# IXarea/LittleGAN

Measured on AMD Instinct MI355X. Metric: 128x128 CelebA-shaped images/sec (G+D+Adj step), higher is better.
Workload: dtype bf16; 1 GPU; C3: 128x128x3 synthetic CelebA, batch 256/GPU, bf16 MFMA conv/transposed-conv + Adjuster branch; global_batch=256, per_gpu_batch=256, image=128, cond_dim=40, parallelism=dp1, launch=eager launches

## Files before the change

### littlegan_amd/csrc/conv_up4.hip

```cpp
#include <type_traits>
#include "lg_internal.h"

namespace {

constexpr int TH = 8, TW = 16, HHT = TH + 2, HWT = TW + 2, NPX = HHT * HWT;
constexpr int KC = 64, KS = KC / 16;
constexpr int PITCH = KC * 2 + 16;
constexpr int HB = 32768;
constexpr int PHW = 10, PNPX = 100, PS1 = 104;
template <bool PAIR> struct U4L {
  static constexpr int HWP = PAIR ? PHW : HWT;
  static constexpr int NPIECE = (PAIR ? 2 * PNPX : NPX) * (KC / 8);
  static constexpr int PPT = (NPIECE + 255) / 256;
};
static_assert((PS1 + PNPX) * PITCH <= HB, "pair halo fits the buffer");
constexpr int SRED_OFF = 2 * HB, SBIAS_OFF = 2 * HB + 256, LDS_BYTES = 2 * HB + 256 + 512;

struct U4Params {
  const __bf16* src;
  const char* wp;
  const float* bias;
  __bf16* out;
  double* spart;
  int B, Hs, Ws, Cs, N, N32, KB;
  int tpi_x, tpi, ntn, nper, nparts;
  int ga, gb;
  LgNormFuse nf;
};

__device__ __forceinline__ int pix32(int r) {
  const int q = r >> 2, lo = r & 3;
  const int odd = (q ^ (q >> 1) ^ (q >> 2)) & 1;
  const int rank = odd ? ((q == 1) ? 0 : (q == 2) ? 1 : (q == 4) ? 2 : 3) : ((q == 0) ? 0 : (q == 3) ? 1 : (q == 5) ? 2 : 3);
  return odd * 16 + rank * 4 + lo;
}

constexpr int nk(int p) { return p ? 3 : 2; }
constexpr int ntaps_of(int cls) { return nk(cls >> 1) * nk(cls & 1); }
constexpr int tap_k(int p, int a) { return p ? 2 * a : 2 * a + 1; }
constexpr int tap_d(int p, int a) { return (p + 1 - tap_k(p, a)) / 2; }
constexpr int tap_widx(int cls, int t) { return tap_k(cls >> 1, t / nk(cls & 1)) * 5 + tap_k(cls & 1, t % nk(cls & 1)); }
constexpr int tap_aoff(int cls, int t, int hwp) {
  return ((tap_d(cls >> 1, t / nk(cls & 1)) + 1) * hwp + tap_d(cls & 1, t % nk(cls & 1)) + 1) * PITCH;
}
template <int CLS, bool STATS, bool FUSE, bool PAIR>
__device__ __forceinline__ void up4_run(const U4Params& p, char* smem, int lb, int G) {
  constexpr int HWP = U4L<PAIR>::HWP, NPIECE = U4L<PAIR>::NPIECE, PPT = U4L<PAIR>::PPT;
  constexpr int F = ntaps_of(CLS) * KS;
  constexpr int RING = F % 8 == 0 ? 8 : 12;
  double* sred = reinterpret_cast<double*>(smem + SRED_OFF);
  float* sbias = reinterpret_cast<float*>(smem + SBIAS_OFF);
  const int tid = threadIdx.x, lane = tid & 63, r = lane & 31, h = lane >> 5;
  const int wid = __builtin_amdgcn_readfirstlane(tid >> 6);
  const int nmine = (p.nper - lb + G - 1) / G;
  const int nchunk = p.Cs / KC;
  const int total = nmine * nchunk;

  int pl[PPT], pyx[PPT];
#pragma unroll
  for (int u = 0; u < PPT; ++u) {
    const int q = tid + u * 256;
    pl[u] = -1; pyx[u] = 0;
    if (q < NPIECE) {
      const int px = q >> 3, pc = q & 7;
      if constexpr (PAIR) {
        const int sl = px >= PNPX, pp = px - PNPX * sl, hy = pp / PHW, hx = pp - hy * PHW;
        pl[u] = (pp + PS1 * sl) * PITCH + pc * 16;
        pyx[u] = (pc << 16) | (hy << 8) | (sl << 7) | hx;
      } else {
        const int hy = px / HWT, hx = px - hy * HWT;
        pl[u] = px * PITCH + pc * 16;
        pyx[u] = (pc << 16) | (hy << 8) | hx;
      }
    }
  }
  int abase[4];
#pragma unroll
  for (int i = 0; i < 4; ++i) {
    const int m = i * 32 + pix32(r);
    const int col = m & 15;
    abase[i] = ((m >> 4) * HWP + (PAIR ? (col & 7) + PS1 * (col >> 3) : col)) * PITCH + h * 16;
  }

  unsigned long long wzero = 0;
  struct Item { int n, y0, x0, tn; };
  auto decode = [&](int k) {
    const int rest = lb + k * G;
    Item it;
    it.tn = rest % p.ntn;
    const int tm = rest / p.ntn;
    if constexpr (PAIR) { it.n = 2 * tm; it.y0 = 0; it.x0 = 0; return it; }
    it.n = tm / p.tpi;
    const int tt = tm - it.n * p.tpi;
    it.y0 = (tt / p.tpi_x) * TH; it.x0 = (tt % p.tpi_x) * TW;
    return it;
  };
  constexpr unsigned OOB = 0x80000000u;
  const int sample_elems = p.Hs * p.Ws * p.Cs;
  auto issue = [&](const Item& it, int c0, u32x4 (&v)[PPT]) {
    const __amdgpu_buffer_rsrc_t rs = __builtin_amdgcn_make_buffer_rsrc(const_cast<__bf16*>(p.src + (long long)it.n * sample_elems), 0,
                                                                        (PAIR ? 2 : 1) * sample_elems * 2, 0x00027000);
#pragma unroll
    for (int u = 0; u < PPT; ++u) {
      const int pq = pyx[u] + (int)wzero;
      const int sy = it.y0 - 1 + ((pq >> 8) & 255), sx = it.x0 - 1 + (pq & (PAIR ? 127 : 255));
      const int sl = PAIR ? (pq >> 7) & 1 : 0;
      const bool in = pl[u] >= 0 && (unsigned)sy < (unsigned)p.Hs && (unsigned)sx < (unsigned)p.Ws;
      const unsigned off = in ? (unsigned)((((sl * p.Hs + sy) * p.Ws + sx) * p.Cs + c0 + (pq >> 16) * 8) * 2) : OOB;
      v[u] = __builtin_bit_cast(u32x4, __builtin_amdgcn_raw_buffer_load_b128(rs, off, 0, 0));
    }
  };
  auto commit = [&](char* buf, const u32x4 (&v)[PPT]) {
#pragma unroll
    for (int u = 0; u < PPT; ++u)
      if (pl[u] >= 0) *reinterpret_cast<u32x4*>(buf + pl[u]) = v[u];
  };
  const unsigned lane16 = lane * 16;
  const unsigned long long wstride = (unsigned long long)p.N32 * p.KB * 1024ull;
  auto wbase = [&](int tn, int kb) { return p.wp + ((long long)(tn * 4 + wid) * p.KB + kb) * 1024; };
  auto wfrag = [&](const char* base, int widx, int ks) {
    return *reinterpret_cast<const u32x4*>((base + ((wzero + (unsigned long long)widx) * wstride + ks * 1024)) + lane16);
  };

  f32x16 acc[4];
#pragma unroll
  for (int i = 0; i < 4; ++i)
#pragma unroll
    for (int e = 0; e < 16; ++e) acc[i][e] = 0.f;
  u32x4 bf[RING];
  u32x4 hv[PPT];

  Item cur = decode(0);
  issue(cur, 0, hv);
  {
    const char* w0 = wbase(cur.tn, 0);
#pragma unroll
    for (int f = 0; f < RING; ++f) bf[f] = wfrag(w0, tap_widx(CLS, f / KS), f % KS);
  }
  commit(smem, hv);
  auto load_bias = [&](int tn) {
    if (tid < 128) sbias[tid] = p.bias ? p.bias[tn * 128 + tid] : 0.f;
  };
  load_bias(cur.tn);
  __syncthreads();

  int k = 0, c = 0;
  Item nxt = cur;
  int c2 = 0;
  auto slice = [&](int s) {
    constexpr int OFF = 0;
    const char* hbuf = smem + (s & 1) * HB;
    const char* wcur = wbase(cur.tn, c * KS);
    const char* wnxt = wbase(nxt.tn, c2 * KS);
    bf16x8 a[2][4];
#pragma unroll
    for (int i = 0; i < 4; ++i) a[0][i] = *reinterpret_cast<const bf16x8*>(hbuf + abase[i] + tap_aoff(CLS, 0, HWP));
    __builtin_amdgcn_sched_barrier(0);
#pragma unroll
    for (int f = 0; f < F; ++f) {
      if (f + 1 < F) {
#pragma unroll
        for (int i = 0; i < 4; ++i)
          a[(f + 1) & 1][i] = *reinterpret_cast<const bf16x8*>(hbuf + abase[i] + tap_aoff(CLS, (f + 1 < F ? f + 1 : 0) / KS, HWP) + ((f + 1) % KS) * 32);
      }
      const int slot = (f + OFF) % RING;
#pragma unroll
      for (int i = 0; i < 4; ++i)
        acc[i] = __builtin_amdgcn_mfma_f32_32x32x16_bf16(__builtin_bit_cast(bf16x8, bf[slot]), a[f & 1][i], acc[i], 0, 0, 0);
      if (f + RING < F) bf[slot] = wfrag(wcur, tap_widx(CLS, (f + RING < F ? f + RING : 0) / KS), (f + RING) % KS);
      else bf[slot] = wfrag(wnxt, tap_widx(CLS, (f + RING >= F ? f + RING - F : 0) / KS), (f + RING - F) % KS);
#pragma unroll
      for (int i = 0; i < 4; ++i) {
        __builtin_amdgcn_sched_group_barrier(0x008, 1, 0);
        __builtin_amdgcn_sched_group_barrier(0x100, 1, 0);
      }
      __builtin_amdgcn_sched_group_barrier(0x020, 1, 0);
    }
    commit(smem + ((s + 1) & 1) * HB, hv);
    __syncthreads();
  };
  auto epilogue = [&](int s, bool more) {
      char* C = smem + (s & 1) * HB;
      const float shift = STATS ? sbias[0] : 0.f;
      const f32x2 shift2 = {shift, shift};
      f32x2 s1v = {0.f, 0.f}, s2v = {0.f, 0.f};
      f32x4 bq[4];
#pragma unroll
      for (int g = 0; g < 4; ++g) bq[g] = *reinterpret_cast<const f32x4*>(sbias + wid * 32 + 8 * g + 4 * h);
#pragma unroll
      for (int i = 0; i < 4; ++i) {
        const int row = i * 32 + pix32(r);
#pragma unroll
        for (int g = 0; g < 4; ++g) {
          bf16x4 w;
#pragma unroll
          for (int jj = 0; jj < 2; ++jj) {
            const f32x2 v = f32x2{acc[i][4 * g + 2 * jj], acc[i][4 * g + 2 * jj + 1]} + f32x2{bq[g][2 * jj], bq[g][2 * jj + 1]};
            if constexpr (STATS) {
              const f32x2 d = v - shift2;
              s1v += d;
              s2v = __builtin_elementwise_fma(d, d, s2v);
            }
            w[2 * jj] = (__bf16)v[0]; w[2 * jj + 1] = (__bf16)v[1];
          }
          *reinterpret_cast<bf16x4*>(C + row * 256 + (((wid * 4 + g) ^ (row & 15)) << 4) + 8 * h) = w;
        }
      }
      if constexpr (STATS) {
        const double l1 = (double)s1v[0] + (double)s1v[1], l2 = (double)s2v[0] + (double)s2v[1];
        if constexpr (PAIR) {
          const bool sb = (pix32(r) & 8) != 0;
          const double a1 = lg_wave_sum_d(sb ? 0.0 : l1), a2 = lg_wave_sum_d(sb ? 0.0 : l2);
          const double b1 = lg_wave_sum_d(sb ? l1 : 0.0), b2 = lg_wave_sum_d(sb ? l2 : 0.0);
          if (lane == 0) {
            double* q = sred + (k & 1) * 16;
            q[wid] = a1; q[4 + wid] = a2; q[8 + wid] = b1; q[12 + wid] = b2;
          }
        } else {
          const double w1 = lg_wave_sum_d(l1), w2 = lg_wave_sum_d(l2);
          if (lane == 0) { sred[(k & 1) * 16 + wid] = w1; sred[(k & 1) * 16 + 4 + wid] = w2; }
        }
      }
      constexpr int py = CLS >> 1, pxc = CLS & 1;
      const long long obase = ((long long)(cur.n * 2 * p.Hs + 2 * cur.y0 + py) * (2 * p.Ws) + 2 * cur.x0 + pxc) * p.N + cur.tn * 128;
      const long long sample_out = (long long)4 * p.Hs * p.Ws * p.N;
      auto pix_off = [&](int row) -> long long {
        if constexpr (PAIR) return obase + ((row >> 3) & 1) * sample_out + ((long long)(2 * (row >> 4)) * (2 * p.Ws) + 2 * (row & 7)) * p.N;
        else return obase + ((long long)(2 * (row >> 4)) * (2 * p.Ws) + 2 * (row & 15)) * p.N;
      };
      u32x4 zq[FUSE ? 8 : 1];
      (void)zq;
      if constexpr (FUSE) {
#pragma unroll
        for (int q8 = 0; q8 < 8; ++q8) {
          const int piece = tid + q8 * 256 + (int)wzero, row = piece >> 4, j = piece & 15;
          zq[q8] = *reinterpret_cast<const u32x4*>(p.nf.z + pix_off(row) + j * 8);
        }
      }
      __syncthreads();
      float nf1 = 0.f, nf2 = 0.f;
      (void)nf1; (void)nf2;
#pragma unroll
      for (int q8 = 0; q8 < 8; ++q8) {
        const int piece = tid + q8 * 256 + (int)wzero, row = piece >> 4, j = piece & 15;
        const u32x4 v = *reinterpret_cast<const u32x4*>(C + row * 256 + ((j ^ (row & 15)) << 4));
        *reinterpret_cast<u32x4*>(p.out + pix_off(row) + j * 8) = v;
        if constexpr (FUSE) {
          const lg_const_f32p sp = lg_as_const(p.nf.stats + (long long)(cur.n + (PAIR ? wid >> 1 : 0)) * 8);
          lg_nf_accum(v, zq[q8], lg_uniform(sp[0]), lg_uniform(sp[4]), lg_uniform(sp[2]), lg_uniform(sp[3]), p.nf.alpha, nf1, nf2);
        }
      }
      if constexpr (FUSE) {
        const double w1 = lg_wave_sum_d((double)nf1), w2 = lg_wave_sum_d((double)nf2);
        if (lane == 0) { sred[(k & 1) * 16 + wid] = w1; sred[(k & 1) * 16 + 4 + wid] = w2; }
      }
      const int tin = PAIR ? 0 : (cur.y0 / TH) * p.tpi_x + cur.x0 / TW;
      const long long prec = (long long)cur.n * p.nparts + (tin * 4 + CLS) * p.ntn + cur.tn;
      if constexpr (STATS) {
        if (tid == 0) {
          const double* q = sred + (k & 1) * 16;
          if constexpr (PAIR) {
            constexpr double cnt = 64.0 * 128.0;
#pragma unroll
            for (int sm = 0; sm < 2; ++sm) {
              const double S1 = (q[8 * sm] + q[8 * sm + 1]) + (q[8 * sm + 2] + q[8 * sm + 3]);
              const double S2 = (q[8 * sm + 4] + q[8 * sm + 5]) + (q[8 * sm + 6] + q[8 * sm + 7]);
              const double md = S1 / cnt;
              double* o = p.spart + (prec + (long long)sm * p.nparts) * 3;
              o[0] = cnt; o[1] = (double)shift + md; o[2] = S2 - cnt * md * md;
            }
          } else {
            constexpr double cnt = 128.0 * 128.0;
            const double S1 = (q[0] + q[1]) + (q[2] + q[3]), S2 = (q[4] + q[5]) + (q[6] + q[7]);
            const double md = S1 / cnt;
            double* o = p.spart + prec * 3;
            o[0] = cnt; o[1] = (double)shift + md; o[2] = S2 - cnt * md * md;
          }
        }
      }
      __syncthreads();
      if constexpr (FUSE) {
        if (tid == 0) {
          const double* q = sred + (k & 1) * 16;
          if constexpr (PAIR) {
#pragma unroll
            for (int sm = 0; sm < 2; ++sm) {
              double* o = p.nf.part + (prec + (long long)sm * p.nparts) * 2;
              o[0] = q[2 * sm] + q[2 * sm + 1]; o[1] = q[4 + 2 * sm] + q[4 + 2 * sm + 1];
            }
          } else {
            double* o = p.nf.part + prec * 2;
            o[0] = (q[0] + q[1]) + (q[2] + q[3]); o[1] = (q[4] + q[5]) + (q[6] + q[7]);
          }
        }
      }
#pragma unroll
      for (int i = 0; i < 4; ++i)
#pragma unroll
        for (int e = 0; e < 16; ++e) acc[i][e] = 0.f;
      if (more && nxt.tn != cur.tn) load_bias(nxt.tn);
      ++k;
  };
  for (int s = 0; s < total; ++s) {
    const bool more = s + 1 < total;
    const bool last_c = c + 1 == nchunk;
    nxt = cur;
    c2 = c + 1;
    if (last_c) { c2 = 0; if (more) nxt = decode(k + 1); }
    if (!more) c2 = c;
    wzero = 0;
    asm volatile("" : "+s"(wzero));
    issue(nxt, c2 * KC, hv);
    slice(s);
    if (last_c) epilogue(s, more);
    cur = nxt;
    c = c2;
  }
}

template <bool STATS, bool FUSE, bool PAIR = false>
__global__ __launch_bounds__(256, 2) void conv_up4_kernel(const U4Params p) {
  static_assert(!(STATS && FUSE), "forward moments and backward sums are never needed together");
  extern __shared__ __attribute__((aligned(16))) char smem[];
  const int b = blockIdx.x;
  if (b < p.ga) {
    up4_run<3, STATS, FUSE, PAIR>(p, smem, b, p.ga);
    __syncthreads();
    up4_run<0, STATS, FUSE, PAIR>(p, smem, b, p.ga);
  } else {
    up4_run<1, STATS, FUSE, PAIR>(p, smem, b - p.ga, p.gb);
    __syncthreads();
    up4_run<2, STATS, FUSE, PAIR>(p, smem, b - p.ga, p.gb);
  }
}

}

enum U4Tiling { U4_NONE = 0, U4_PLAIN, U4_PAIR };
static U4Tiling up4_tiling(int B, int Hm, int Wm, int Cs, int N) {
  static int off = -1;
  if (off < 0) off = lg_env_flag("LG_NO_UP4") ? 1 : 0;
  if (off || B <= 0 || Cs % KC || N % 128) return U4_NONE;
  if ((long long)Hm * Wm * Cs * 2 * 2 >= (1ll << 31)) return U4_NONE;
  if (Hm == 8 && Wm == 8 && B % 2 == 0) return U4_PAIR;
  return (Hm % TH == 0 && Wm % TW == 0) ? U4_PLAIN : U4_NONE;
}
extern "C" int lg_conv_up4_supported(int B, int Hm, int Wm, int Cs, int N) { return up4_tiling(B, Hm, Wm, Cs, N) != U4_NONE ? 1 : 0; }

extern "C" int lg_conv_up4_nf_try(const void* src16, const void* wpack_up, const float* bias, void* out16, int B, int Hm, int Wm,
                                  int Cs, int N, void* spart, size_t spart_bytes, int* nparts_out, const LgNormFuse* nf,
                                  size_t nf_bytes, void* stream) {
  if (nparts_out) *nparts_out = 0;
  const U4Tiling tiling = up4_tiling(B, Hm, Wm, Cs, N);
  if (tiling == U4_NONE || !src16 || !wpack_up || !out16) return LG_ERR_UNSUPPORTED;
  const bool pair = tiling == U4_PAIR;
  U4Params p{};
  p.src = (const __bf16*)src16; p.wp = (const char*)wpack_up; p.bias = bias; p.out = (__bf16*)out16;
  p.B = B; p.Hs = Hm; p.Ws = Wm; p.Cs = Cs; p.N = N; p.N32 = N / 32; p.KB = Cs / 16;
  p.tpi_x = pair ? 1 : Wm / TW; p.tpi = pair ? 1 : p.tpi_x * (Hm / TH); p.ntn = N / 128;
  const long long nper = (long long)(pair ? B / 2 : B) * p.tpi * p.ntn;
  if (nper <= 0 || 4 * nper >= (1ll << 30)) return LG_ERR_UNSUPPORTED;
  p.nper = (int)nper; p.nparts = p.tpi * 4 * p.ntn;
  const bool fuse = nf && nf->z && nf->stats && nf->part && nparts_out && (size_t)B * p.nparts * 2 * sizeof(double) <= nf_bytes;
  const bool stats = !fuse && spart && nparts_out && (size_t)B * p.nparts * 3 * sizeof(double) <= spart_bytes;
  if (!nf && spart && nparts_out && !stats) return LG_ERR_UNSUPPORTED;
  p.spart = stats ? (double*)spart : nullptr;
  if (fuse) p.nf = *nf;
  static bool attr_set = false;
  const int nblk = 2 * lg_grid_cus();
  if (!attr_set) {
    attr_set = true;
    (void)hipFuncSetAttribute(reinterpret_cast<const void*>((conv_up4_kernel<true, false>)), hipFuncAttributeMaxDynamicSharedMemorySize, LDS_BYTES);
    (void)hipFuncSetAttribute(reinterpret_cast<const void*>((conv_up4_kernel<false, false>)), hipFuncAttributeMaxDynamicSharedMemorySize, LDS_BYTES);
    (void)hipFuncSetAttribute(reinterpret_cast<const void*>((conv_up4_kernel<false, true>)), hipFuncAttributeMaxDynamicSharedMemorySize, LDS_BYTES);
    (void)hipFuncSetAttribute(reinterpret_cast<const void*>((conv_up4_kernel<true, false, true>)), hipFuncAttributeMaxDynamicSharedMemorySize, LDS_BYTES);
    (void)hipFuncSetAttribute(reinterpret_cast<const void*>((conv_up4_kernel<false, false, true>)), hipFuncAttributeMaxDynamicSharedMemorySize, LDS_BYTES);
    (void)hipFuncSetAttribute(reinterpret_cast<const void*>((conv_up4_kernel<false, true, true>)), hipFuncAttributeMaxDynamicSharedMemorySize, LDS_BYTES);
  }
  long long best = -1;
  p.ga = p.gb = 1;
  for (int ga = 1; ga < nblk && ga <= p.nper; ++ga) {
    int gb = nblk - ga;
    if (gb > p.nper) gb = p.nper;
    if (gb < 1) break;
    const long long ca = (long long)((p.nper + ga - 1) / ga) * 13, cb = (long long)((p.nper + gb - 1) / gb) * 12;
    const long long cost = (ca > cb ? ca : cb) * 4096 - (ga + gb);
    if (best < 0 || cost < best) { best = cost; p.ga = ga; p.gb = gb; }
  }
  const int grid = p.ga + p.gb;
  hipStream_t st = (hipStream_t)stream;
  if (pair) {
    if (fuse) hipLaunchKernelGGL((conv_up4_kernel<false, true, true>), dim3(grid), dim3(256), LDS_BYTES, st, p);
    else if (stats) hipLaunchKernelGGL((conv_up4_kernel<true, false, true>), dim3(grid), dim3(256), LDS_BYTES, st, p);
    else hipLaunchKernelGGL((conv_up4_kernel<false, false, true>), dim3(grid), dim3(256), LDS_BYTES, st, p);
  } else if (fuse) hipLaunchKernelGGL((conv_up4_kernel<false, true>), dim3(grid), dim3(256), LDS_BYTES, st, p);
  else if (stats) hipLaunchKernelGGL((conv_up4_kernel<true, false>), dim3(grid), dim3(256), LDS_BYTES, st, p);
  else hipLaunchKernelGGL((conv_up4_kernel<false, false>), dim3(grid), dim3(256), LDS_BYTES, st, p);
  LG_CHECK_LAUNCH("lg_conv_up4");
  lg_note_kernel(pair ? "conv_up4_kernel<PAIR>" : "conv_up4_kernel");
  if (stats || fuse) *nparts_out = p.nparts;
  return LG_OK;
}
extern "C" int lg_conv_up4_try(const void* src16, const void* wpack_up, const float* bias, void* out16, int B, int Hm, int Wm,
                               int Cs, int N, void* spart, size_t spart_bytes, int* nparts_out, void* stream) {
  return lg_conv_up4_nf_try(src16, wpack_up, bias, out16, B, Hm, Wm, Cs, N, spart, spart_bytes, nparts_out, nullptr, 0, stream);
}
```

Before: 25050 images/sec.

## Store conv_up4 epilogue directly from registers via permlane32 swap

For non-fused variants (pair or no-stats), the epilogue now packs bf16 results in registers, exchanges halves across lanes with permlane32_swap, and writes 16-byte global stores directly, bypassing the LDS staging round-trip and its barriers. Bias is double-buffered in LDS so the next tile's bias is prefetched without a sync, and the per-tile moment records are written one slice later (deferred flush) instead of behind an extra barrier. The exchange costs extra LDS space and register pressure, and stores are less coalesced per instruction than the LDS-transposed path.

```diff
diff --git a/littlegan_amd/csrc/conv_up4.hip b/littlegan_amd/csrc/conv_up4.hip
--- a/littlegan_amd/csrc/conv_up4.hip
+++ b/littlegan_amd/csrc/conv_up4.hip
@@ -14,7 +14,11 @@
   static constexpr int PPT = (NPIECE + 255) / 256;
 };
 static_assert((PS1 + PNPX) * PITCH <= HB, "pair halo fits the buffer");
-constexpr int SRED_OFF = 2 * HB, SBIAS_OFF = 2 * HB + 256, LDS_BYTES = 2 * HB + 256 + 512;
+constexpr int SRED_OFF = 2 * HB, SBIAS_OFF = 2 * HB + 256, LDS_BYTES = 2 * HB + 256 + 1024;
+typedef unsigned u4_u32x2 __attribute__((ext_vector_type(2)));
+
+template <bool STATS, bool FUSE, bool PAIR>
+constexpr bool u4_reg_epilogue() { return !FUSE && (PAIR || !STATS); }
 
 struct U4Params {
   const __bf16* src;
@@ -147,6 +151,36 @@
   int k = 0, c = 0;
   Item nxt = cur;
   int c2 = 0;
+  constexpr bool REGEPI = u4_reg_epilogue<STATS, FUSE, PAIR>();
+  static_assert(!(REGEPI && FUSE), "the fused sums leave through the LDS epilogue");
+  int bv = 0;
+  bool pend = false;
+  long long prec_p = 0;
+  float pshift = 0.f;
+  (void)bv; (void)pend; (void)prec_p; (void)pshift;
+  auto flush_record = [&]() {
+    if (tid == 0) {
+      const double* q = sred + ((k - 1) & 1) * 16;
+      if constexpr (STATS && PAIR) {
+        constexpr double cnt = 64.0 * 128.0;
+#pragma unroll
+        for (int sm = 0; sm < 2; ++sm) {
+          const double S1 = (q[8 * sm] + q[8 * sm + 1]) + (q[8 * sm + 2] + q[8 * sm + 3]);
+          const double S2 = (q[8 * sm + 4] + q[8 * sm + 5]) + (q[8 * sm + 6] + q[8 * sm + 7]);
+          const double md = S1 / cnt;
+          double* o = p.spart + (prec_p + (long long)sm * p.nparts) * 3;
+          o[0] = cnt; o[1] = (double)pshift + md; o[2] = S2 - cnt * md * md;
+        }
+      } else if constexpr (STATS) {
+        constexpr double cnt = 128.0 * 128.0;
+        const double S1 = (q[0] + q[1]) + (q[2] + q[3]), S2 = (q[4] + q[5]) + (q[6] + q[7]);
+        const double md = S1 / cnt;
+        double* o = p.spart + prec_p * 3;
+        o[0] = cnt; o[1] = (double)pshift + md; o[2] = S2 - cnt * md * md;
+      }
+    }
+    pend = false;
+  };
   auto slice = [&](int s) {
     constexpr int OFF = 0;
     const char* hbuf = smem + (s & 1) * HB;
@@ -178,6 +212,84 @@
     }
     commit(smem + ((s + 1) & 1) * HB, hv);
     __syncthreads();
+  };
+  auto epilogue_reg = [&](bool more) {
+      const float* sb = sbias + bv * 128;
+      const float shift = STATS ? sb[0] : 0.f;
+      const f32x2 shift2 = {shift, shift};
+      f32x2 s1v = {0.f, 0.f}, s2v = {0.f, 0.f};
+      f32x4 bq[4];
+#pragma unroll
+      for (int g = 0; g < 4; ++g) bq[g] = *reinterpret_cast<const f32x4*>(sb + wid * 32 + 8 * g + 4 * h);
+      const bool newb = more && nxt.tn != cur.tn;
+      float bnext = 0.f;
+      if (newb && tid < 128 && p.bias) bnext = p.bias[nxt.tn * 128 + tid];
+      constexpr int py = CLS >> 1, pxc = CLS & 1;
+      const long long obase = ((long long)(cur.n * 2 * p.Hs + 2 * cur.y0 + py) * (2 * p.Ws) + 2 * cur.x0 + pxc) * p.N + cur.tn * 128;
+      const long long sample_out = (long long)4 * p.Hs * p.Ws * p.N;
+      auto pix_off = [&](int row) -> long long {
+        if constexpr (PAIR) return obase + ((row >> 3) & 1) * sample_out + ((long long)(2 * (row >> 4)) * (2 * p.Ws) + 2 * (row & 7)) * p.N;
+        else return obase + ((long long)(2 * (row >> 4)) * (2 * p.Ws) + 2 * (row & 15)) * p.N;
+      };
+      const int coff = wid * 32 + 8 * h;
+#pragma unroll
+      for (int i = 0; i < 4; ++i) {
+        const long long goff = pix_off(i * 32 + pix32(r)) + coff;
+#pragma unroll
+        for (int gp = 0; gp < 2; ++gp) {
+          u4_u32x2 ab[2];
+#pragma unroll
+          for (int gg = 0; gg < 2; ++gg) {
+            const int g = 2 * gp + gg;
+            bf16x4 w;
+#pragma unroll
+            for (int jj = 0; jj < 2; ++jj) {
+              const f32x2 v = f32x2{acc[i][4 * g + 2 * jj], acc[i][4 * g + 2 * jj + 1]} + f32x2{bq[g][2 * jj], bq[g][2 * jj + 1]};
+              if constexpr (STATS) {
+                const f32x2 d = v - shift2;
+                s1v += d;
+                s2v = __builtin_elementwise_fma(d, d, s2v);
+              }
+              w[2 * jj] = (__bf16)v[0]; w[2 * jj + 1] = (__bf16)v[1];
+            }
+            ab[gg] = __builtin_bit_cast(u4_u32x2, w);
+          }
+          const auto x = __builtin_amdgcn_permlane32_swap(ab[0][0], ab[1][0], false, false);
+          const auto y = __builtin_amdgcn_permlane32_swap(ab[0][1], ab[1][1], false, false);
+          const u32x4 v = {x[0], y[0], x[1], y[1]};
+          *reinterpret_cast<u32x4*>(p.out + goff + 16 * gp) = v;
+        }
+      }
+      if constexpr (STATS) {
+        const double l1 = (double)s1v[0] + (double)s1v[1], l2 = (double)s2v[0] + (double)s2v[1];
+        if constexpr (PAIR) {
+          const bool sb1 = (pix32(r) & 8) != 0;
+          const double a1 = lg_wave_sum_d(sb1 ? 0.0 : l1), a2 = lg_wave_sum_d(sb1 ? 0.0 : l2);
+          const double b1 = lg_wave_sum_d(sb1 ? l1 : 0.0), b2 = lg_wave_sum_d(sb1 ? l2 : 0.0);
+          if (lane == 0) {
+            double* q = sred + (k & 1) * 16;
+            q[wid] = a1; q[4 + wid] = a2; q[8 + wid] = b1; q[12 + wid] = b2;
+          }
+        } else {
+          const double w1 = lg_wave_sum_d(l1), w2 = lg_wave_sum_d(l2);
+          if (lane == 0) { sred[(k & 1) * 16 + wid] = w1; sred[(k & 1) * 16 + 4 + wid] = w2; }
+        }
+      }
+      if constexpr (STATS) {
+        const int tin = PAIR ? 0 : (cur.y0 / TH) * p.tpi_x + cur.x0 / TW;
+        prec_p = (long long)cur.n * p.nparts + (tin * 4 + CLS) * p.ntn + cur.tn;
+        pshift = shift;
+        pend = true;
+      }
+#pragma unroll
+      for (int i = 0; i < 4; ++i)
+#pragma unroll
+        for (int e = 0; e < 16; ++e) acc[i][e] = 0.f;
+      if (newb) {
+        bv ^= 1;
+        if (tid < 128) sbias[bv * 128 + tid] = bnext;
+      }
+      ++k;
   };
   auto epilogue = [&](int s, bool more) {
       char* C = smem + (s & 1) * HB;
@@ -312,9 +424,19 @@
     asm volatile("" : "+s"(wzero));
     issue(nxt, c2 * KC, hv);
     slice(s);
-    if (last_c) epilogue(s, more);
+    if constexpr (REGEPI && STATS) {
+      if (pend) flush_record();
+    }
+    if (last_c) {
+      if constexpr (REGEPI) epilogue_reg(more);
+      else epilogue(s, more);
+    }
     cur = nxt;
     c = c2;
+  }
+  if constexpr (REGEPI && STATS) {
+    __syncthreads();
+    if (pend) flush_record();
   }
 }
 
diff --git a/profiles/regepi_conv_up4_moments_pair_new.s b/profiles/regepi_conv_up4_moments_pair_new.s
--- /dev/null
+++ b/profiles/regepi_conv_up4_moments_pair_new.s
@@ -0,0 +1,163 @@
+	v_lshl_add_u64 v[176:177], v[134:135], 1, v[50:51]
+	s_waitcnt lgkmcnt(1)
+	v_add_f32_e32 v59, v59, v103
+	v_add_f32_e32 v58, v58, v102
+	v_add_f32_e32 v56, v61, v105
+	v_add_f32_e32 v57, v60, v104
+	s_waitcnt lgkmcnt(0)
+	v_add_f32_e32 v54, v63, v99
+	v_add_f32_e32 v55, v62, v98
+	v_add_f32_e32 v50, v65, v101
+	v_add_f32_e32 v51, v64, v100
+	v_cvt_pk_bf16_f32 v61, v57, v56
+	v_cvt_pk_bf16_f32 v60, v58, v59
+	v_cvt_pk_bf16_f32 v63, v51, v50
+	v_cvt_pk_bf16_f32 v62, v55, v54
+	v_cvt_pk_bf16_f32 v123, v118, v117
+	v_cvt_pk_bf16_f32 v122, v120, v119
+	v_cvt_pk_bf16_f32 v125, v53, v52
+	v_cvt_pk_bf16_f32 v124, v116, v115
+	v_permlane32_swap_b32_e32 v60, v62
+	v_permlane32_swap_b32_e32 v61, v63
+	v_permlane32_swap_b32_e32 v122, v124
+	v_permlane32_swap_b32_e32 v123, v125
+	global_store_dwordx4 v[176:177], v[60:63], off offset:32
+	global_store_dwordx4 v[176:177], v[122:125], off
+	s_nop 0
+	v_mov_b32_e32 v60, v139
+	s_and_saveexec_b64 s[94:95], s[0:1]
+	s_cbranch_execz .LBB3_137
+	v_cmp_lt_i32_e32 vcc, 1, v133
+	s_mov_b64 s[96:97], 0
+	s_and_saveexec_b64 s[50:51], vcc
+	s_xor_b64 s[98:99], exec, s[50:51]
+	s_cbranch_execnz .LBB3_167
+	s_or_saveexec_b64 s[98:99], s[98:99]
+	v_mov_b32_e32 v60, 4
+	s_xor_b64 exec, exec, s[98:99]
+	s_cbranch_execnz .LBB3_170
+.LBB3_134:
+	s_or_b64 exec, exec, s[98:99]
+	s_and_saveexec_b64 s[80:81], s[96:97]
+.LBB3_135:
+	v_mov_b32_e32 v60, v138
+.LBB3_136:
+	s_or_b64 exec, exec, s[80:81]
+.LBB3_137:
+	s_or_b64 exec, exec, s[94:95]
+	v_add_u32_e32 v60, v60, v147
+	v_add_u32_e32 v61, 32, v60
+	v_bfe_u32 v62, v60, 3, 1
+	v_lshrrev_b32_e32 v61, 3, v61
+	v_lshlrev_b32_e32 v60, 1, v60
+	v_mul_lo_u32 v177, s85, v62
+	v_mul_lo_u32 v176, s84, v62
+	v_and_b32_e32 v61, 14, v61
+	v_and_b32_e32 v136, 14, v60
+	v_mad_i64_i32 v[60:61], s[50:51], v61, s16, v[136:137]
+	v_add_f32_e32 v64, v35, v111
+	v_add_f32_e32 v65, v34, v110
+	v_lshl_add_u64 v[34:35], v[176:177], 1, s[46:47]
+	v_mul_lo_u32 v61, v61, s18
+	v_mul_lo_u32 v62, v60, s17
+	v_mad_u64_u32 v[178:179], s[50:51], v60, s18, 0
+	v_lshl_add_u64 v[34:35], s[36:37], 1, v[34:35]
+	v_add3_u32 v179, v179, v62, v61
+	v_lshl_add_u64 v[34:35], s[92:93], 1, v[34:35]
+	v_lshl_add_u64 v[34:35], v[178:179], 1, v[34:35]
+	v_add_f32_e32 v62, v37, v113
+	v_add_f32_e32 v63, v36, v112
+	v_add_f32_e32 v60, v39, v107
+	v_add_f32_e32 v61, v38, v106
+	v_add_f32_e32 v36, v41, v109
+	v_add_f32_e32 v37, v40, v108
+	v_lshl_add_u64 v[176:177], v[134:135], 1, v[34:35]
+	v_add_f32_e32 v43, v43, v103
+	v_add_f32_e32 v42, v42, v102
+	v_add_f32_e32 v40, v45, v105
+	v_add_f32_e32 v41, v44, v104
+	v_add_f32_e32 v38, v47, v99
+	v_add_f32_e32 v39, v46, v98
+	v_add_f32_e32 v34, v49, v101
+	v_add_f32_e32 v35, v48, v100
+	v_cvt_pk_bf16_f32 v45, v41, v40
+	v_cvt_pk_bf16_f32 v44, v42, v43
+	v_cvt_pk_bf16_f32 v47, v35, v34
+	v_cvt_pk_bf16_f32 v46, v39, v38
+	v_cvt_pk_bf16_f32 v123, v63, v62
+	v_cvt_pk_bf16_f32 v122, v65, v64
+	v_cvt_pk_bf16_f32 v125, v37, v36
+	v_cvt_pk_bf16_f32 v124, v61, v60
+	v_permlane32_swap_b32_e32 v44, v46
+	v_permlane32_swap_b32_e32 v45, v47
+	v_permlane32_swap_b32_e32 v122, v124
+	v_permlane32_swap_b32_e32 v123, v125
+	global_store_dwordx4 v[176:177], v[44:47], off offset:32
+	global_store_dwordx4 v[176:177], v[122:125], off
+	s_nop 0
+	v_mov_b32_e32 v44, v139
+	s_and_saveexec_b64 s[94:95], s[0:1]
+	s_cbranch_execz .LBB3_143
+	v_cmp_lt_i32_e32 vcc, 1, v133
+	s_mov_b64 s[96:97], 0
+	s_and_saveexec_b64 s[50:51], vcc
+	s_xor_b64 s[98:99], exec, s[50:51]
+	s_cbranch_execnz .LBB3_171
+	s_or_saveexec_b64 s[98:99], s[98:99]
+	v_mov_b32_e32 v44, 4
+	s_xor_b64 exec, exec, s[98:99]
+	s_cbranch_execnz .LBB3_174
+.LBB3_140:
+	s_or_b64 exec, exec, s[98:99]
+	s_and_saveexec_b64 s[80:81], s[96:97]
+.LBB3_141:
+	v_mov_b32_e32 v44, v138
+.LBB3_142:
+	s_or_b64 exec, exec, s[80:81]
+.LBB3_143:
+	s_or_b64 exec, exec, s[94:95]
+	v_add_u32_e32 v44, v44, v147
+	v_or_b32_e32 v45, 64, v44
+	v_bfe_u32 v46, v44, 3, 1
+	v_lshrrev_b32_e32 v45, 3, v45
+	v_lshlrev_b32_e32 v44, 1, v44
+	v_mul_lo_u32 v177, s85, v46
+	v_mul_lo_u32 v176, s84, v46
+	v_and_b32_e32 v45, 14, v45
+	v_and_b32_e32 v136, 14, v44
+	v_mad_i64_i32 v[44:45], s[50:51], v45, s16, v[136:137]
+	v_add_f32_e32 v48, v19, v111
+	v_add_f32_e32 v49, v18, v110
+	v_lshl_add_u64 v[18:19], v[176:177], 1, s[46:47]
+	v_mul_lo_u32 v45, v45, s18
+	v_mul_lo_u32 v46, v44, s17
+	v_mad_u64_u32 v[178:179], s[50:51], v44, s18, 0
+	v_lshl_add_u64 v[18:19], s[36:37], 1, v[18:19]
+	v_add3_u32 v179, v179, v46, v45
+	v_lshl_add_u64 v[18:19], s[92:93], 1, v[18:19]
+	v_lshl_add_u64 v[18:19], v[178:179], 1, v[18:19]
+	v_add_f32_e32 v46, v21, v113
+	v_add_f32_e32 v47, v20, v112
+	v_add_f32_e32 v44, v23, v107
+	v_add_f32_e32 v45, v22, v106
+	v_add_f32_e32 v20, v25, v109
+	v_add_f32_e32 v21, v24, v108
+	v_lshl_add_u64 v[176:177], v[134:135], 1, v[18:19]
+	v_add_f32_e32 v27, v27, v103
+	v_add_f32_e32 v26, v26, v102
+	v_add_f32_e32 v24, v29, v105
+	v_add_f32_e32 v25, v28, v104
+	v_add_f32_e32 v22, v31, v99
+	v_add_f32_e32 v23, v30, v98
+	v_add_f32_e32 v18, v33, v101
+	v_add_f32_e32 v19, v32, v100
+	v_cvt_pk_bf16_f32 v29, v25, v24
+	v_cvt_pk_bf16_f32 v28, v26, v27
+	v_cvt_pk_bf16_f32 v31, v19, v18
+	v_cvt_pk_bf16_f32 v30, v23, v22
+	v_cvt_pk_bf16_f32 v123, v47, v46
+	v_cvt_pk_bf16_f32 v122, v49, v48
+	v_cvt_pk_bf16_f32 v125, v21, v20
+	v_cvt_pk_bf16_f32 v124, v45, v44
+	v_permlane32_swap_b32_e32 v28, v30
+	v_permlane32_swap_b32_e32 v29, v31
diff --git a/profiles/regepi_conv_up4_moments_pair_parent.s b/profiles/regepi_conv_up4_moments_pair_parent.s
--- /dev/null
+++ b/profiles/regepi_conv_up4_moments_pair_parent.s
@@ -0,0 +1,226 @@
+	v_xor_b32_e32 v52, s10, v52
+	v_cvt_pk_bf16_f32 v51, v116, v115
+	v_cvt_pk_bf16_f32 v50, v120, v119
+	v_add3_u32 v52, v122, v52, v152
+	ds_write_b64 v52, v[50:51]
+	v_bitop3_b32 v52, v121, s11, 15 bitop3:0x6c
+	s_waitcnt lgkmcnt(3)
+	v_add_f32_e32 v117, v55, v107
+	v_add_f32_e32 v118, v54, v106
+	v_add_f32_e32 v57, v57, v109
+	v_add_f32_e32 v56, v56, v108
+	v_lshlrev_b32_e32 v52, 4, v52
+	v_cvt_pk_bf16_f32 v51, v56, v57
+	v_cvt_pk_bf16_f32 v50, v118, v117
+	v_add3_u32 v52, v122, v52, v152
+	v_bitop3_b32 v54, v121, s12, 15 bitop3:0x6c
+	ds_write_b64 v52, v[50:51]
+	s_waitcnt lgkmcnt(3)
+	v_add_f32_e32 v59, v59, v103
+	v_add_f32_e32 v58, v58, v102
+	v_add_f32_e32 v52, v61, v105
+	v_add_f32_e32 v53, v60, v104
+	v_lshlrev_b32_e32 v54, 4, v54
+	v_cvt_pk_bf16_f32 v51, v53, v52
+	v_cvt_pk_bf16_f32 v50, v58, v59
+	v_add3_u32 v54, v122, v54, v152
+	s_waitcnt lgkmcnt(2)
+	v_add_f32_e32 v55, v62, v98
+	v_bitop3_b32 v62, v121, s13, 15 bitop3:0x6c
+	ds_write_b64 v54, v[50:51]
+	v_add_f32_e32 v54, v63, v99
+	v_add_f32_e32 v50, v65, v101
+	v_add_f32_e32 v51, v64, v100
+	v_lshlrev_b32_e32 v62, 4, v62
+	v_cvt_pk_bf16_f32 v61, v51, v50
+	v_cvt_pk_bf16_f32 v60, v55, v54
+	v_add3_u32 v62, v122, v62, v152
+	ds_write_b64 v62, v[60:61]
+	v_mov_b32_e32 v60, v140
+	s_and_saveexec_b64 s[36:37], s[0:1]
+	s_cbranch_execz .LBB3_129
+	v_cmp_lt_i32_e32 vcc, 1, v138
+	s_mov_b64 s[92:93], 0
+	s_and_saveexec_b64 s[94:95], vcc
+	s_xor_b64 s[94:95], exec, s[94:95]
+	s_cbranch_execnz .LBB3_164
+	s_or_saveexec_b64 s[94:95], s[94:95]
+	v_mov_b32_e32 v60, 4
+	s_xor_b64 exec, exec, s[94:95]
+	s_cbranch_execnz .LBB3_167
+.LBB3_126:
+	s_or_b64 exec, exec, s[94:95]
+	s_and_saveexec_b64 s[94:95], s[92:93]
+.LBB3_127:
+	v_mov_b32_e32 v60, v139
+.LBB3_128:
+	s_or_b64 exec, exec, s[94:95]
+.LBB3_129:
+	s_or_b64 exec, exec, s[36:37]
+	v_add_u32_e32 v121, v60, v150
+	v_and_b32_e32 v62, 15, v121
+	v_add_f32_e32 v61, v36, v112
+	v_lshlrev_b32_e32 v36, 4, v62
+	v_lshl_add_u32 v122, v121, 8, s78
+	v_add_f32_e32 v64, v35, v111
+	v_add_f32_e32 v65, v34, v110
+	v_add_f32_e32 v60, v37, v113
+	v_xor_b32_e32 v36, s10, v36
+	v_cvt_pk_bf16_f32 v35, v61, v60
+	v_cvt_pk_bf16_f32 v34, v65, v64
+	v_add3_u32 v36, v122, v36, v152
+	s_lshl_b64 s[36:37], s[36:37], 1
+	s_waitcnt lgkmcnt(0)
+	s_barrier
+	ds_read_b128 v[2:5], v2
+	v_mul_lo_u32 v11, v9, s72
+	v_mul_lo_u32 v12, v8, s17
+	v_mad_u64_u32 v[8:9], s[94:95], v8, s72, 0
+	v_lshl_add_u64 v[6:7], v[6:7], 0, s[36:37]
+	s_lshl_b64 s[92:93], s[92:93], 1
+	v_add3_u32 v9, v9, v12, v11
+	v_lshl_add_u64 v[6:7], v[6:7], 0, s[92:93]
+	v_lshl_add_u64 v[6:7], v[8:9], 1, v[6:7]
+	v_lshlrev_b32_e32 v8, 4, v10
+	v_and_b32_e32 v134, 0xf0, v8
+	v_add_u32_e32 v11, s90, v143
+	v_lshl_add_u64 v[6:7], v[6:7], 0, v[134:135]
+	v_ashrrev_i32_e32 v8, 4, v11
+	s_waitcnt lgkmcnt(0)
+	global_store_dwordx4 v[6:7], v[2:5], off
+	v_bfe_u32 v6, v8, 3, 1
+	v_ashrrev_i32_e32 v9, 7, v11
+	v_xor_b32_e32 v3, v8, v11
+	v_lshlrev_b32_e32 v2, 8, v8
+	v_lshlrev_b32_e32 v3, 4, v3
+	v_lshlrev_b32_e32 v8, 1, v8
+	v_and_b32_e32 v3, 0xf0, v3
+	v_mul_lo_u32 v7, s83, v6
+	v_mul_lo_u32 v6, s82, v6
+	v_and_b32_e32 v9, -2, v9
+	v_and_b32_e32 v134, 14, v8
+	v_add3_u32 v2, s78, v2, v3
+	v_mad_i64_i32 v[8:9], s[94:95], v9, s16, v[134:135]
+	v_lshl_add_u64 v[6:7], v[6:7], 1, s[46:47]
+	ds_read_b128 v[2:5], v2
+	v_mul_lo_u32 v12, v9, s72
+	v_mul_lo_u32 v13, v8, s17
+	v_mad_u64_u32 v[8:9], s[94:95], v8, s72, 0
+	v_lshl_add_u64 v[6:7], v[6:7], 0, s[36:37]
+	v_add3_u32 v9, v9, v13, v12
+	v_lshl_add_u64 v[6:7], v[6:7], 0, s[92:93]
+	v_lshl_add_u64 v[6:7], v[8:9], 1, v[6:7]
+	v_lshlrev_b32_e32 v8, 4, v11
+	v_and_b32_e32 v134, 0xf0, v8
+	v_add_u32_e32 v11, s90, v146
+	v_lshl_add_u64 v[6:7], v[6:7], 0, v[134:135]
+	v_ashrrev_i32_e32 v8, 4, v11
+	s_waitcnt lgkmcnt(0)
+	global_store_dwordx4 v[6:7], v[2:5], off
+	v_bfe_u32 v6, v8, 3, 1
+	v_ashrrev_i32_e32 v9, 7, v11
+	v_xor_b32_e32 v3, v8, v11
+	v_lshlrev_b32_e32 v2, 8, v8
+	v_lshlrev_b32_e32 v3, 4, v3
+	v_lshlrev_b32_e32 v8, 1, v8
+	v_and_b32_e32 v3, 0xf0, v3
+	v_mul_lo_u32 v7, s83, v6
+	v_mul_lo_u32 v6, s82, v6
+	v_and_b32_e32 v9, -2, v9
+	v_and_b32_e32 v134, 14, v8
+	v_add3_u32 v2, s78, v2, v3
+	v_mad_i64_i32 v[8:9], s[94:95], v9, s16, v[134:135]
+	v_lshl_add_u64 v[6:7], v[6:7], 1, s[46:47]
+	ds_read_b128 v[2:5], v2
+	v_mul_lo_u32 v12, v9, s72
+	v_mul_lo_u32 v13, v8, s17
+	v_mad_u64_u32 v[8:9], s[94:95], v8, s72, 0
+	v_lshl_add_u64 v[6:7], v[6:7], 0, s[36:37]
+	v_add3_u32 v9, v9, v13, v12
+	v_lshl_add_u64 v[6:7], v[6:7], 0, s[92:93]
+	v_lshl_add_u64 v[6:7], v[8:9], 1, v[6:7]
+	v_lshlrev_b32_e32 v8, 4, v11
+	v_and_b32_e32 v134, 0xf0, v8
+	v_add_u32_e32 v11, s90, v131
+	v_lshl_add_u64 v[6:7], v[6:7], 0, v[134:135]
+	v_ashrrev_i32_e32 v8, 4, v11
+	s_waitcnt lgkmcnt(0)
+	global_store_dwordx4 v[6:7], v[2:5], off
+	v_bfe_u32 v6, v8, 3, 1
+	v_ashrrev_i32_e32 v9, 7, v11
+	v_xor_b32_e32 v3, v8, v11
+	v_lshlrev_b32_e32 v2, 8, v8
+	v_lshlrev_b32_e32 v3, 4, v3
+	v_lshlrev_b32_e32 v8, 1, v8
+	v_and_b32_e32 v3, 0xf0, v3
+	v_mul_lo_u32 v7, s83, v6
+	v_mul_lo_u32 v6, s82, v6
+	v_and_b32_e32 v9, -2, v9
+	v_and_b32_e32 v134, 14, v8
+	v_add3_u32 v2, s78, v2, v3
+	v_mad_i64_i32 v[8:9], s[94:95], v9, s16, v[134:135]
+	v_lshl_add_u64 v[6:7], v[6:7], 1, s[46:47]
+	ds_read_b128 v[2:5], v2
+	v_mul_lo_u32 v12, v9, s72
+	v_mul_lo_u32 v13, v8, s17
+	v_mad_u64_u32 v[8:9], s[94:95], v8, s72, 0
+	v_lshl_add_u64 v[6:7], v[6:7], 0, s[36:37]
+	v_add3_u32 v9, v9, v13, v12
+	v_lshl_add_u64 v[6:7], v[6:7], 0, s[92:93]
+	v_lshl_add_u64 v[6:7], v[8:9], 1, v[6:7]
+	v_lshlrev_b32_e32 v8, 4, v11
+	v_and_b32_e32 v134, 0xf0, v8
+	v_add_u32_e32 v11, s90, v133
+	v_lshl_add_u64 v[6:7], v[6:7], 0, v[134:135]
+	v_ashrrev_i32_e32 v8, 4, v11
+	s_waitcnt lgkmcnt(0)
+	global_store_dwordx4 v[6:7], v[2:5], off
+	v_bfe_u32 v6, v8, 3, 1
+	v_ashrrev_i32_e32 v9, 7, v11
+	v_xor_b32_e32 v3, v8, v11
+	v_lshlrev_b32_e32 v2, 8, v8
+	v_lshlrev_b32_e32 v3, 4, v3
+	v_lshlrev_b32_e32 v8, 1, v8
+	v_and_b32_e32 v3, 0xf0, v3
+	v_mul_lo_u32 v7, s83, v6
+	v_mul_lo_u32 v6, s82, v6
+	v_and_b32_e32 v9, -2, v9
+	v_and_b32_e32 v134, 14, v8
+	v_add3_u32 v2, s78, v2, v3
+	v_mad_i64_i32 v[8:9], s[94:95], v9, s16, v[134:135]
+	v_lshl_add_u64 v[6:7], v[6:7], 1, s[46:47]
+	ds_read_b128 v[2:5], v2
+	v_mul_lo_u32 v12, v9, s72
+	v_mul_lo_u32 v13, v8, s17
+	v_mad_u64_u32 v[8:9], s[94:95], v8, s72, 0
+	v_lshl_add_u64 v[6:7], v[6:7], 0, s[36:37]
+	v_add3_u32 v9, v9, v13, v12
+	v_lshl_add_u64 v[6:7], v[6:7], 0, s[92:93]
+	v_lshl_add_u64 v[6:7], v[8:9], 1, v[6:7]
+	v_lshlrev_b32_e32 v8, 4, v11
+	v_and_b32_e32 v134, 0xf0, v8
+	v_add_u32_e32 v11, s90, v136
+	v_lshl_add_u64 v[6:7], v[6:7], 0, v[134:135]
+	v_ashrrev_i32_e32 v8, 4, v11
+	s_waitcnt lgkmcnt(0)
+	global_store_dwordx4 v[6:7], v[2:5], off
+	v_bfe_u32 v6, v8, 3, 1
+	v_ashrrev_i32_e32 v9, 7, v11
+	v_xor_b32_e32 v3, v8, v11
+	v_lshlrev_b32_e32 v2, 8, v8
+	v_lshlrev_b32_e32 v3, 4, v3
+	v_lshlrev_b32_e32 v8, 1, v8
+	v_and_b32_e32 v3, 0xf0, v3
+	v_mul_lo_u32 v7, s83, v6
+	v_mul_lo_u32 v6, s82, v6
+	v_and_b32_e32 v9, -2, v9
+	v_and_b32_e32 v134, 14, v8
+	v_add3_u32 v2, s78, v2, v3
+	v_mad_i64_i32 v[8:9], s[94:95], v9, s16, v[134:135]
+	v_lshl_add_u64 v[6:7], v[6:7], 1, s[46:47]
+	ds_read_b128 v[2:5], v2
+	v_mul_lo_u32 v12, v9, s72
+	v_mul_lo_u32 v13, v8, s17
+	v_mad_u64_u32 v[8:9], s[94:95], v8, s72, 0
+	v_lshl_add_u64 v[6:7], v[6:7], 0, s[36:37]
+	v_add3_u32 v9, v9, v13, v12
```

After: 25040 images/sec (median of 2 runs). About the same (-0.0%).
